# MarwanMousa/MARL-for-IM

Hardware: NVIDIA B200
Metric: agent_steps_per_sec (higher is better)
Workload: dtype i32 state / f64 obs+reward

## Files before the change

### marl_for_im_b200/csrc/imx_api.cu

```cuda
#include <cmath>
#include <cstdarg>
#include <cstdio>
#include <cstdlib>
#include <cstring>
#include <atomic>
#include <new>
#include <vector>

#include <nvtx3/nvToolsExt.h>

#include "imx_reset.cuh"
#include "imx_step_tma.cuh"
#include "imx_rollout.cuh"
#include "imx_step_pipe.cuh"
#include "imx_rollout_et.cuh"
#include "imx_kernels.cuh"
#include "imx_stats.cuh"
#include "imx_jit.cuh"
#include "imx_cc.cuh"
#include "imx_eval.cuh"

using namespace imx;

static thread_local char g_err[512] = "";
// ... 34 lines not shown
        a.message.ascii = name;
        return &a;
    }
};
#define IMX_NVTX(name) NvtxRange nvtx_range__(name)

extern "C" const char* imx_last_error(void) { return g_err; }
extern "C" int imx_abi_version(void) { return IMX_ABI_VERSION; }
extern "C" int imx_config_size(void) { return (int)sizeof(imx_config); }
extern "C" int64_t imx_launch_count(void) { return g_launches.load(); }

typedef void (*reset_fn_t)(const StepArgs, const ResetArgs, int);

struct imx_env {
    imx_config cfg;
    bool div, multi;
    int m, T, P, D, O, L, NB, R, maxc;
    int demand_max[IMX_MAX_NODES];
    int depth[IMX_MAX_NODES], parent[IMX_MAX_NODES], child_slot[IMX_MAX_NODES];
    int retailers[IMX_MAX_NODES], retailer_idx[IMX_MAX_NODES];
    double sell[IMX_MAX_NODES], buy[IMX_MAX_NODES];
    bool need_hd, need_ho, write_hd, has_carry;
    int S;
    int64_t N;
    NodeParams* d_nodes = nullptr;
    int32_t* d_state = nullptr;
    size_t state_bytes = 0;
    void* field_ptr[IMX_F_COUNT] = {};
    int64_t field_cnt[IMX_F_COUNT] = {};
    int32_t* d_err = nullptr;
    int32_t* d_demand_T = nullptr;
    uint8_t* d_mask_T = nullptr;
    double* d_cdf = nullptr;
    uint16_t* d_guide = nullptr;
    int cdf_len = 0;
    double* d_stats_partial = nullptr;
    double* d_dfo_rewards = nullptr;
    double* d_tab = nullptr;
    int TL = 0;
    cudaStream_t hstream = nullptr;
    double *d_act_h = nullptr, *d_obs_h = nullptr, *d_rew_h = nullptr;
    int32_t* d_dem_h = nullptr;
    uint8_t* d_mask_h = nullptr;
    int t = 0;
    int noisy_now = 0;
    uint64_t episode = 0;
    step_fn_t step_fn = nullptr;
    tma_fn_t tma_fn = nullptr;
    tma_fn_t tma_many_fn = nullptr;
    TileLayout tile = {};
    TileLayout tile_jit = {};
    int step_path = 0;
    int host_zero_copy = 1;
    int step_dense = 0;
    int tma_threads = 256;
    int use_pdl = 1;
    int fuse_periods = 1;
    int l2_hints = 0;
    int step_et = 0;
    int rollout_et = 0;
    int jit_threads = 128;
    int pipe_mode = 0;
    int pipe_stages = 0;
    int pipe_ctas = 0;
    int sm_count = 148;
    int jit_policy = 0;
    int jit_state = 0;
    const imxjit::Kernels* jit = nullptr;
    const imxjit::Kernels* jit_noobs = nullptr;
    int jit_noobs_state = 0;
    const imxjit::Kernels* jit_cc = nullptr;
    int jit_cc_state = 0;
    TileLayout tile_cc = {};
    void* d_obs_scratch = nullptr;
    const imxjit::Kernels* jit_ep = nullptr;
    const imxjit::Kernels* jit_ep_noobs = nullptr;
    int jit_ep_state = 0, jit_ep_noobs_state = 0;
    double* d_ep_rewards = nullptr;
    double* d_ep_profit = nullptr;
    double* d_ep_ret = nullptr;
    double* d_ep_stats = nullptr;
    int last_variant = 0;
    reset_fn_t reset_fn = nullptr;
    rollout_fn_t rollout_fn = nullptr;
    int step_grid_cap = 0, rollout_grid_cap = 0;
    size_t step_smem = 0;
    int m_pad = 0;
};

static int obs_type_of(const imx_config& c) { return (c.io_flags & IMX_IO_OBS_BF16) ? OBS_BF16 : c.obs_f32 ? OBS_F32 : OBS_F64; }
static int obs_elem_bytes(const imx_env* e) { return imx::obs_elem_bytes(obs_type_of(e->cfg)); }
static int act_elem_bytes(const imx_env* e) { return (e->cfg.io_flags & IMX_IO_ACTIONS_F32) ? 4 : 8; }
static int64_t bytes_per_env(const imx_env* e) {
    return 8 * (int64_t)e->S + 4 * e->R + (int64_t)e->m * (act_elem_bytes(e) + 8 + e->O * obs_elem_bytes(e));
}

#define IMX_DECL_PICK(MP, DV) void imx_pick_kernels_##MP##_##DV(bool small, bool few, imx::KernelSet* ks);
IMX_DECL_PICK(2, 0) IMX_DECL_PICK(4, 0) IMX_DECL_PICK(8, 0) IMX_DECL_PICK(16, 0) IMX_DECL_PICK(32, 0)
IMX_DECL_PICK(4, 1) IMX_DECL_PICK(8, 1) IMX_DECL_PICK(16, 1) IMX_DECL_PICK(32, 1)
#undef IMX_DECL_PICK

static int m_pad_of(const imx_env* e);
static void pick_kernels(imx_env* e, int m_pad, bool div) {
    const bool small = (e->D <= 4 && e->P <= 1);
    const bool few = e->maxc <= 2;
    KernelSet ks;
    if (div) {
        if (m_pad == 4) imx_pick_kernels_4_1(small, few, &ks);
        else if (m_pad == 8) imx_pick_kernels_8_1(small, few, &ks);
        else if (m_pad == 16) imx_pick_kernels_16_1(small, few, &ks);
        else imx_pick_kernels_32_1(small, few, &ks);
    } else {
        if (m_pad == 2) imx_pick_kernels_2_0(small, few, &ks);
        else if (m_pad == 4) imx_pick_kernels_4_0(small, few, &ks);
        else if (m_pad == 8) imx_pick_kernels_8_0(small, few, &ks);
        else if (m_pad == 16) imx_pick_kernels_16_0(small, few, &ks);
        else imx_pick_kernels_32_0(small, few, &ks);
    }
    e->step_fn = ks.step_fn; e->tma_fn = ks.tma_fn; e->tma_many_fn = ks.tma_many_fn; e->rollout_fn = ks.rollout_fn;
    const int ot = obs_type_of(e->cfg);
    if (ot == OBS_BF16) e->reset_fn = small ? reset_kernel<4, 1, OBS_BF16> : reset_kernel<8, 8, OBS_BF16>;
    else if (ot == OBS_F32) e->reset_fn = small ? reset_kernel<4, 1, OBS_F32> : reset_kernel<8, 8, OBS_F32>;
    else e->reset_fn = small ? reset_kernel<4, 1, OBS_F64> : reset_kernel<8, 8, OBS_F64>;
    e->m_pad = m_pad;
}

static cudaError_t raise_dyn_smem_limit(const void* fn, size_t bytes) {
    cudaFuncAttributes fa;
    cudaError_t rc = cudaFuncGetAttributes(&fa, fn);
    if (rc != cudaSuccess) return rc;
    if ((size_t)fa.maxDynamicSharedSizeBytes >= bytes) return cudaSuccess;
    return cudaFuncSetAttribute(fn, cudaFuncAttributeMaxDynamicSharedMemorySize, (int)bytes);
}

static int m_pad_of(const imx_env* e);

static int choose_tma_threads(const imx_env* e) {
    const char* tt = getenv("IMX_TMA_THREADS");
    const bool small4 = !e->div && m_pad_of(e) == 4 && e->N >= 1024 && bytes_per_env(e) * e->N <= ((int64_t)192 << 20);
    const bool big4 = !e->div && m_pad_of(e) == 4 && e->N >= ((int64_t)1 << 19);
    const int dflt = small4 ? 64 : (big4 || (m_pad_of(e) <= 4 && e->N >= ((int64_t)1 << 20))) ? 256 : 128;
    const int v = tt ? atoi(tt) : dflt;
    return ((v == 64 || v == 128 || v == 256 || v == 512) && v >= 2 * m_pad_of(e)) ? v : 256;
}

static int m_pad_of(const imx_env* e) {
    const int m = e->m;
    if (e->div) return m <= 4 ? 4 : m <= 8 ? 8 : m <= 16 ? 16 : 32;
    return m <= 2 ? 2 : m <= 4 ? 4 : m <= 8 ? 8 : m <= 16 ? 16 : 32;
}

static void compute_tile(const imx_env* e, TileLayout& L, int tile_width, bool with_cc = false, int E_fixed = 0) {
    const int m = e->m;
    const int E = E_fixed > 0 ? E_fixed : (e->tma_threads / 32) * (32 / tile_width);
    int off = 0;
    auto take = [&](int bytes) { const int o = off; off += (bytes + 127) & ~127; return o; };
    L.E = E;
    const int act_region = E * m * (act_elem_bytes(e) == 4 ? 12 : 8);
    L.off_act = take(act_region);
    L.off_inv = take(E * m * 4);
    L.off_bl = take(E * m * 4);
    L.off_ou = take(E * m * 4);
    L.off_pipe = take(E * e->L * 4);
    L.off_hd = take(e->need_hd ? E * m * e->P * 4 : 0);
    L.off_ho = take(e->need_ho ? E * m * e->P * 4 : 0);
    L.off_carry = take(e->has_carry ? E * m * 4 : 0);
// ... 646 lines not shown
            IMX_CREATE_CUDA(cudaMemcpy(reinterpret_cast<float*>(e->d_tab + tab.size()) + tab.size(), tabh.data(), tab.size() * sizeof(uint16_t),
                                       cudaMemcpyHostToDevice));
        }
    }
    {
        const int cols = e->multi ? m : 1;
        const int64_t nslices = (N + stats_envs_per_block(cols) - 1) / stats_envs_per_block(cols);
        const size_t a = (size_t)(2 + 2 * cols) * (size_t)nslices, b = (size_t)(2 * EVAL_FIXED + 2 + 2 * IMX_MAX_NODES) * STATS_BLOCKS;
        IMX_CREATE_CUDA(cudaMalloc(&e->d_stats_partial, (a > b ? a : b) * sizeof(double)));
    }
    IMX_CREATE_CUDA(cudaMemset(e->d_demand_T, 0, dem_bytes));
    {
        launch_reset_kernel(e, nullptr, nullptr);
        cudaError_t le = cudaGetLastError();
        if (le != cudaSuccess) { fail(-3, "reset launch failed: %s", cudaGetErrorString(le)); imx_destroy(e); return -3; }
        g_launches.fetch_add(1);
        IMX_CREATE_CUDA(cudaDeviceSynchronize());
    }
#undef IMX_CREATE_CUDA
    ensure_jit(e);
    *out = e;
    return 0;
}

extern "C" int imx_destroy(imx_env* e) {
    if (!e) return 0;
    cudaSetDevice(e->cfg.device);
    if (e->hstream) { cudaStreamSynchronize(e->hstream); cudaStreamDestroy(e->hstream); }
    cudaFree(e->d_nodes); cudaFree(e->d_state); cudaFree(e->d_err);
    cudaFree(e->d_demand_T); cudaFree(e->d_mask_T); cudaFree(e->d_cdf); cudaFree(e->d_guide); cudaFree(e->d_tab); cudaFree(e->d_stats_partial);
    cudaFree(e->d_dfo_rewards); cudaFree(e->d_obs_scratch);
    cudaFree(e->d_ep_rewards); cudaFree(e->d_ep_profit); cudaFree(e->d_ep_ret); cudaFree(e->d_ep_stats);
    cudaFree(e->d_act_h); cudaFree(e->d_obs_h); cudaFree(e->d_rew_h); cudaFree(e->d_dem_h); cudaFree(e->d_mask_h);
    delete e;
    return 0;
}

extern "C" int imx_obs_len(const imx_env* e) { return e ? e->O : fail(-1, "null env"); }
extern "C" int imx_state_words(const imx_env* e) { return e ? e->S : fail(-1, "null env"); }
extern "C" int imx_num_retailers(const imx_env* e) { return e ? e->R : fail(-1, "null env"); }
extern "C" int imx_pipe_words(const imx_env* e) { return e ? e->L : fail(-1, "null env"); }
extern "C" int imx_ledger_words(const imx_env* e) { return e ? e->NB : fail(-1, "null env"); }
extern "C" int imx_retailers(const imx_env* e, int32_t* out) {
    if (!e || !out) return fail(-1, "null argument");
    for (int k = 0; k < e->R; ++k) out[k] = e->retailers[k];
    return 0;
}
extern "C" int imx_demand_max(const imx_env* e, int32_t* out) {
    if (!e || !out) return fail(-1, "null argument");
    for (int i = 0; i < e->m; ++i) out[i] = e->demand_max[i];
    return 0;
}
extern "C" int imx_node_price(const imx_env* e, double* sell, double* buy) {
    if (!e || !sell || !buy) return fail(-1, "null argument");
    for (int i = 0; i < e->m; ++i) { sell[i] = e->sell[i]; buy[i] = e->buy[i]; }
    return 0;
}
extern "C" int imx_state_field(imx_env* e, int field, void** dev_ptr, int64_t* count) {
    if (!e || !dev_ptr || !count) return fail(-1, "null argument");
    if (field < 0 || field >= IMX_F_COUNT) return fail(-1, "unknown field %d", field);
    *dev_ptr = e->field_ptr[field];
    *count = e->field_cnt[field];
    return 0;
}
extern "C" int imx_period(const imx_env* e) { return e ? e->t : fail(-1, "null env"); }
extern "C" int imx_set_period(imx_env* e, int t) {
    if (!e) return fail(-1, "null env");
    if (t < 0 || t > e->T) return fail(-1, "period %d outside [0, %d]", t, e->T);
    e->t = t;
    return 0;
}

static void launch_reset_kernel(imx_env* e, double* obs_dev, cudaStream_t s, const int32_t* demand_in) {
    StepArgs A;
    fill_args(e, A);
    A.obs = obs_dev;
    ResetArgs Z;
    Z.zero_base = e->d_state;
    Z.zero_words = (int64_t)(e->state_bytes / sizeof(int32_t));
    Z.err = e->d_err;
    Z.demand_in = demand_in;
    Z.demand_T = e->d_demand_T;
    Z.R = e->R; Z.T = e->T;
    const int64_t work = (obs_dev ? e->N * e->m * e->O : 0) > Z.zero_words / 4 ? e->N * e->m * e->O : Z.zero_words / 4;
    int sms = 148;
    cudaDeviceGetAttribute(&sms, cudaDevAttrMultiProcessorCount, e->cfg.device);
    int64_t blocks = (work + 255) / 256;
    if (blocks > (int64_t)sms * 8) blocks = (int64_t)sms * 8;
    if (blocks < 1) blocks = 1;
    const size_t smem = (size_t)e->m * e->O * sizeof(double) + (size_t)e->m * sizeof(int32_t);
    cudaLaunchConfig_t lc;
    memset(&lc, 0, sizeof(lc));
    lc.gridDim = dim3((unsigned)blocks); lc.blockDim = dim3(256); lc.dynamicSmemBytes = smem; lc.stream = s;
    cudaLaunchAttribute at[1];
    at[0].id = cudaLaunchAttributeProgrammaticStreamSerialization;
    at[0].val.programmaticStreamSerializationAllowed = 1;
    lc.attrs = at;
    lc.numAttrs = e->use_pdl ? 1 : 0;
    cudaLaunchKernelEx(&lc, e->reset_fn, A, Z, e->div ? 1 : 0);
}

static DemandGen make_gen(const imx_env* e, uint64_t episode) {
    DemandGen g;
    g.dist = e->cfg.demand_dist; g.low = e->cfg.uniform_low; g.high = e->cfg.uniform_high;
    g.cdf_len = e->cdf_len; g.cdf = e->d_cdf; g.guide = e->d_guide; g.seed = e->cfg.seed; g.episode = episode; g.env_offset = e->cfg.env_offset;
    g.noise_thr = e->div ? e->cfg.noisy_demand_threshold : 0.0;
    return g;
}

extern "C" int imx_reset(imx_env* e, const int32_t* demand_dev, const uint8_t* delay_mask_dev, int noisy,
                         uint64_t episode, void* obs_dev, void* stream) {
    IMX_NVTX("imx_reset");

    if (!e) return fail(-1, "null env");
    cudaStream_t s = (cudaStream_t)stream;
    IMX_CUDA(cudaSetDevice(e->cfg.device));
    if ((noisy || delay_mask_dev) && !e->has_carry) return fail(-1, "noisy delay requested but the env was created with noisy_delay = 0");
    if (!demand_dev && e->cfg.demand_dist == IMX_DIST_REPLAY_ONLY)
        return fail(-1, "reset() without a demand trace needs demand_dist poisson or uniform");
    const int64_t N = e->N;
    const unsigned gb = (unsigned)((N * e->R + 255) / 256);
    if (!demand_dev) {
        demand_generate_kernel<<<gb, 256, 0, s>>>(e->d_demand_T, N, e->R, e->T, make_gen(e, episode));
        IMX_CHECK_LAUNCH("demand_generate_kernel");
    }
    e->noisy_now = (noisy || delay_mask_dev) ? 1 : 0;
    const int64_t cells = N * e->m;
    const unsigned cb = (unsigned)((cells + 255) / 256);
    if (e->noisy_now) {
        if (delay_mask_dev) {
            mask_transpose_kernel<<<cb, 256, 0, s>>>(delay_mask_dev, e->d_mask_T, N, e->m, e->T);
            IMX_CHECK_LAUNCH("mask_transpose_kernel");
        } else {
            mask_generate_kernel<<<cb, 256, 0, s>>>(e->d_mask_T, N, e->m, e->T, e->cfg.seed, e->cfg.env_offset, episode,
                                                    e->cfg.noisy_delay_threshold);
            IMX_CHECK_LAUNCH("mask_generate_kernel");
        }
    }
    e->t = 0;
    e->episode = episode;
    launch_reset_kernel(e, (double*)obs_dev, s, demand_dev);
    IMX_CHECK_LAUNCH("reset_kernel");
    return 0;
}

static bool pipe_pays(const imx_env* e, int n_tiles) {
    (void)n_tiles;
    if (e->step_et) return bytes_per_env(e) * e->N <= ((int64_t)384 << 20);
    if (e->div) return true;
    if (e->l2_hints) return true;
    return bytes_per_env(e) * e->N <= ((int64_t)192 << 20);
}
static int pipe_ctas_for(const imx_env* e, const TileLayout& L) {
    const bool is_cc = (&L == &e->tile_cc);
    int want = 4;
    if (e->pipe_ctas > 0) want = e->pipe_ctas;
    else if (e->step_et && !is_cc) want = 6;
    else if (e->div) want = m_pad_of(e) <= 4 ? 4 : 6;
    else if (e->jit_threads == 64) want = 8;
    const int64_t per_cta = (int64_t)pipe_stages_for(e, L) * L.total + 1024 + 256;
    const int fit = (int)((228 * 1024) / per_cta);
    if (want > fit) want = fit;
    return want < 1 ? 1 : want;
}

struct CcOut { void* dev; int fill; double lo, hi; };
static bool tile_io_whole16(const imx_env* e, const TileLayout& L, bool cc) {
    const int64_t cells = (int64_t)L.E * e->m;
    if ((cells * act_elem_bytes(e)) % 16 != 0 || (cells * e->O * obs_elem_bytes(e)) % 16 != 0) return false;
    return !cc || (cells * ((e->m - 1) * (1 + e->O) + e->O) * obs_elem_bytes(e)) % 16 == 0;
}
constexpr unsigned ET_THREADS_HOST = 128;

// ... 329 lines not shown
        return fail(-1, "rollout without a demand trace needs demand_dist poisson or uniform");
    if ((noisy || delay_mask_dev) && !e->has_carry) return fail(-1, "noisy delay requested but the env was created with noisy_delay = 0");
    cudaStream_t s = (cudaStream_t)stream;
    IMX_CUDA(cudaSetDevice(e->cfg.device));
    if (dfo_dev && !step_reward_dev) {
        if (!e->d_dfo_rewards) {
            if (stream_is_capturing(s)) return fail(-1, "dfo_dev without step_reward_dev under stream capture: call imx_prepare(IMX_PREPARE_DFO) first");
            IMX_CUDA(cudaMalloc(&e->d_dfo_rewards, (size_t)e->T * e->N * sizeof(double)));
        }
        step_reward_dev = e->d_dfo_rewards;
    }
    StepArgs A;
    fill_args(e, A);
    A.t = 0;
    RolloutArgs Rg;
    memset(&Rg, 0, sizeof(Rg));
    Rg.z = z_dev; Rg.z_stride = z_stride; Rg.demand = demand_dev;
    Rg.ret = return_dev; Rg.step_reward = step_reward_dev; Rg.write_state = write_state;
    Rg.mask = delay_mask_dev; Rg.noisy = (noisy || delay_mask_dev) ? 1 : 0; Rg.delay_thr = e->cfg.noisy_delay_threshold;
    Rg.gen = make_gen(e, episode);
    const int epw = 32 / e->m_pad;
    const size_t draw_bytes = (size_t)(ROLLOUT_THREADS / 32) * epw * e->R * ((e->T + 1) & ~1) * sizeof(int32_t);
    const bool coop = (!demand_dev && draw_bytes <= 40 * 1024);
    Rg.coop_demand = coop ? 1 : 0;
    const size_t roll_smem = coop ? draw_bytes : 0;
    const int64_t warp_tiles = (e->N + epw - 1) / epw;
    const int64_t blocks_needed = (warp_tiles + (ROLLOUT_THREADS / 32) - 1) / (ROLLOUT_THREADS / 32);
    const unsigned grid = (unsigned)(blocks_needed < e->rollout_grid_cap ? blocks_needed : e->rollout_grid_cap);
    if (e->jit_state == 1 && e->jit->rollout && e->rollout_et) {
        EtNodeConsts C;
        memset(&C, 0, sizeof(C));
        for (int i = 0; i < e->m; ++i) {
            C.p[i] = e->sell[i]; C.c[i] = e->buy[i]; C.h[i] = e->cfg.stock_cost[i]; C.bc[i] = e->cfg.backlog_cost[i]; C.target[i] = e->cfg.inv_target[i];
        }
        void* params[] = {(void*)&A, (void*)&Rg, (void*)&C};
        const int64_t blocks = (e->N + ET_THREADS_HOST - 1) / ET_THREADS_HOST;
        const int64_t cap = (int64_t)e->sm_count * 16;
        Rg.coop_demand = 0;
        const CUresult cr = imxjit::g_api.LaunchKernel(e->jit->rollout, (unsigned)(blocks < cap ? blocks : cap), 1, 1, ET_THREADS_HOST, 1, 1, 0, (CUstream)s,
                                                       params, nullptr);
        if (cr != CUDA_SUCCESS) return fail(-3, "launch of the env-per-thread rollout kernel failed (CUresult %d)", (int)cr);
        g_launches.fetch_add(1, std::memory_order_relaxed);
        e->last_variant = 2;
    } else if (e->jit_state == 1 && e->jit->rollout) {
        void* params[] = {(void*)&A, (void*)&Rg};
        const int epw_j = 32 / e->m;
        const int64_t wt_j = (e->N + epw_j - 1) / epw_j;
        const int64_t need_j = (wt_j + (ROLLOUT_THREADS / 32) - 1) / (ROLLOUT_THREADS / 32);
        const int64_t cap_j = (int64_t)e->rollout_grid_cap * 4;
        const unsigned g2 = (unsigned)(need_j < cap_j ? need_j : cap_j);
        const size_t draw_j = (size_t)(ROLLOUT_THREADS / 32) * epw_j * e->R * ((e->T + 1) & ~1) * sizeof(int32_t);
        if (coop && draw_j > 40 * 1024) Rg.coop_demand = 0;
        const size_t roll_smem_j = Rg.coop_demand ? draw_j : 0;
        const CUresult cr = imxjit::g_api.LaunchKernel(e->jit->rollout, g2, 1, 1, ROLLOUT_THREADS, 1, 1, (unsigned)roll_smem_j, (CUstream)s, params, nullptr);
        if (cr != CUDA_SUCCESS) return fail(-3, "launch of the specialised rollout kernel failed (CUresult %d)", (int)cr);
        g_launches.fetch_add(1, std::memory_order_relaxed);
        e->last_variant = 2;
    } else {
        e->rollout_fn<<<grid, ROLLOUT_THREADS, roll_smem, s>>>(A, Rg);
        IMX_CHECK_LAUNCH("rollout_kernel");
        e->last_variant = 0;
    }
    if (dfo_dev) {
        dfo_objective_kernel<<<(unsigned)((e->N + 127) / 128), 128, 0, s>>>(pmf_dev, step_reward_dev, dfo_dev, e->N, e->R, e->T);
        IMX_CHECK_LAUNCH("dfo_objective_kernel");
    }
    if (write_state) { e->t = e->T; e->episode = episode; e->noisy_now = Rg.noisy; }
    return 0;
}

template <typename... KArgs, typename... Args>
static cudaError_t launch_dependent(void (*kern)(KArgs...), dim3 grid, dim3 block, cudaStream_t s, bool pdl, Args... args) {
    cudaLaunchConfig_t lc;
    memset(&lc, 0, sizeof(lc));
    lc.gridDim = grid; lc.blockDim = block; lc.dynamicSmemBytes = 0; lc.stream = s;
    cudaLaunchAttribute at[1];
    at[0].id = cudaLaunchAttributeProgrammaticStreamSerialization;
    at[0].val.programmaticStreamSerializationAllowed = 1;
    lc.attrs = at;
    lc.numAttrs = pdl ? 1 : 0;
    return cudaLaunchKernelEx(&lc, kern, KArgs(args)...);
}

static int launch_return_stats(imx_env* e, const double* src, int periods, bool fused, double* ret_out, double* stats_dev, int accumulate,
                               cudaStream_t s) {
    const int cols = e->multi ? e->m : 1;
    const int per_agent = e->multi ? 1 : 0;
    const int nstat = per_agent ? 2 + 2 * cols : 2;
    const int epb = stats_envs_per_block(cols);
    const int nslices = (int)((e->N + epb - 1) / epb);
    const bool pdl = e->use_pdl != 0;
    if (fused && periods == 1 && !ret_out) fused = false;
    if (fused)
        IMX_CUDA(launch_dependent(stats_slice_kernel<true>, dim3((unsigned)nslices), dim3(STATS_THREADS), s, pdl, src, ret_out, e->d_stats_partial,
                                  e->N, cols, per_agent, periods, epb, nslices));
    else
        IMX_CUDA(launch_dependent(stats_slice_kernel<false>, dim3((unsigned)nslices), dim3(STATS_THREADS), s, pdl, src, (double*)nullptr,
                                  e->d_stats_partial, e->N, cols, per_agent, 1, epb, nslices));
    g_launches.fetch_add(1, std::memory_order_relaxed);
    IMX_CUDA(launch_dependent(stats_final_kernel, dim3((unsigned)nstat), dim3(STATS_THREADS), s, pdl, (const double*)e->d_stats_partial, stats_dev,
                              e->N, nslices, accumulate));
    g_launches.fetch_add(1, std::memory_order_relaxed);
    return 0;
}

extern "C" int imx_return_stats(imx_env* e, const double* return_dev, double* stats_dev, void* stream) {
    if (!e || !return_dev || !stats_dev) return fail(-1, "null argument");
    IMX_CUDA(cudaSetDevice(e->cfg.device));
    return launch_return_stats(e, return_dev, 1, false, nullptr, stats_dev, 0, (cudaStream_t)stream);
}

extern "C" int imx_episode_stats(imx_env* e, const double* step_reward_dev, int periods, double* return_dev, double* stats_dev,
                                 int accumulate, void* stream) {
    IMX_NVTX("imx_episode_stats");

    if (!e || !step_reward_dev || !stats_dev) return fail(-1, "null argument");
    if (periods < 1) return fail(-1, "periods must be >= 1");
    IMX_CUDA(cudaSetDevice(e->cfg.device));
    return launch_return_stats(e, step_reward_dev, periods, true, return_dev, stats_dev, accumulate, (cudaStream_t)stream);
}

extern "C" int imx_eval_len(const imx_env* e) { return e ? EVAL_FIXED + e->m : -1; }

extern "C" int imx_eval_accumulate(imx_env* e, const void* obs_dev, const double* reward_dev, const double* profit_dev,
                                   double* acc_dev, int reset, void* stream) {
    if (!e || !obs_dev || !reward_dev || !acc_dev) return fail(-1, "null argument");
    IMX_CUDA(cudaSetDevice(e->cfg.device));
    EvalArgs E;
    memset(&E, 0, sizeof(E));
    E.obs = obs_dev; E.reward = reward_dev; E.profit = profit_dev; E.acc = acc_dev; E.nodes = e->d_nodes;
    E.N = e->N; E.m = e->m; E.O = e->O; E.multi = e->multi ? 1 : 0; E.obs_type = obs_type_of(e->cfg);
    E.rescaled = (e->cfg.kind == IMX_KIND_MAIM_DIV || e->cfg.standardise_state) ? 1 : 0;
    E.reset = reset ? 1 : 0;
    E.a = e->cfg.a; E.bma = e->cfg.b - e->cfg.a;
    eval_accumulate_kernel<<<(unsigned)((e->N + 255) / 256), 256, 0, (cudaStream_t)stream>>>(E);
    IMX_CHECK_LAUNCH("eval_accumulate_kernel");
    return 0;
}

extern "C" int imx_eval_stats(imx_env* e, const double* acc_dev, double* stats_dev, int accumulate, void* stream) {
    if (!e || !acc_dev || !stats_dev) return fail(-1, "null argument");
    IMX_CUDA(cudaSetDevice(e->cfg.device));
    const int W = EVAL_FIXED + e->m;
    column_stats_partial_kernel<<<dim3(STATS_BLOCKS, 2 * W), STATS_THREADS, 0, (cudaStream_t)stream>>>(acc_dev, e->d_stats_partial, e->N, W);
    IMX_CHECK_LAUNCH("column_stats_partial_kernel");
    stats_final_kernel<<<2 * W, STATS_THREADS, 0, (cudaStream_t)stream>>>(e->d_stats_partial, stats_dev, e->N, STATS_BLOCKS, accumulate);
    IMX_CHECK_LAUNCH("stats_final_kernel");
    return 0;
}

static int ensure_host_path(imx_env* e) {
    if (e->hstream) return 0;
    const size_t cells = (size_t)e->N * e->m;
    cudaError_t rc = cudaSuccess;
    auto take = [&](void** p, size_t bytes) { if (rc == cudaSuccess && !*p) rc = cudaMalloc(p, bytes); };
    take((void**)&e->d_act_h, cells * sizeof(double));
    take((void**)&e->d_obs_h, cells * e->O * obs_elem_bytes(e));
    take((void**)&e->d_rew_h, cells * sizeof(double));
    take((void**)&e->d_dem_h, (size_t)e->N * e->R * e->T * sizeof(int32_t));
    if (e->has_carry) take((void**)&e->d_mask_h, (size_t)e->N * e->T * e->m);
    cudaStream_t hs = nullptr;
    if (rc == cudaSuccess) rc = cudaStreamCreateWithFlags(&hs, cudaStreamNonBlocking);
    if (rc != cudaSuccess) {
        cudaFree(e->d_act_h); cudaFree(e->d_obs_h); cudaFree(e->d_rew_h); cudaFree(e->d_dem_h); cudaFree(e->d_mask_h);
        e->d_act_h = e->d_obs_h = e->d_rew_h = nullptr; e->d_dem_h = nullptr; e->d_mask_h = nullptr;
        return fail(-2, "host-path staging allocation failed: %s", cudaGetErrorString(rc));
    }
    e->hstream = hs;
    return 0;
}

extern "C" int imx_reset_host(imx_env* e, const int32_t* demand_host, const uint8_t* delay_mask_host, int noisy,
                              uint64_t episode, void* obs_host) {
    IMX_NVTX("imx_reset_host");

    if (!e) return fail(-1, "null env");
    IMX_CUDA(cudaSetDevice(e->cfg.device));
    int rc = ensure_host_path(e);
    if (rc) return rc;
    cudaStream_t s = e->hstream;
    if (demand_host)
// ... 140 lines not shown
```

### marl_for_im_b200/csrc/imx_reset.cuh

```cuda
#pragma once

#include "imx_step.cuh"

namespace imx {

struct ResetArgs {
    int32_t* zero_base;
    int64_t zero_words;
    int32_t* err;
    const int32_t* demand_in;
    int32_t* demand_T;
    int32_t R, T;
};
constexpr int RESET_T_CHUNK = 8;

template <int DMAX, int PMAX, int OT>
__global__ void __launch_bounds__(256) reset_kernel(const __grid_constant__ StepArgs A_, const __grid_constant__ ResetArgs Z, int div) {
    extern __shared__ __align__(16) double s_tmpl[];
    StepArgs A = A_;
    A.obs_type = OT;
    const int m = A.m, O = A.O;
    const int es = obs_elem_bytes(OT);
    int32_t* s_init = reinterpret_cast<int32_t*>(s_tmpl + m * O);
    asm volatile("griddepcontrol.wait;" ::: "memory");
    asm volatile("griddepcontrol.launch_dependents;" ::: "memory");
    if ((int)threadIdx.x < m) {
        const int i = threadIdx.x;
        const NodeParams np = load_node(A.nodes + i);
        s_init[i] = np.init_inv;
        if (A.obs) {
            int pipe[DMAX], hd[PMAX], ho[PMAX];
#pragma unroll
            for (int k = 0; k < DMAX; ++k) pipe[k] = 0;
#pragma unroll
            for (int j = 0; j < PMAX; ++j) { hd[j] = 0; ho[j] = 0; }
            write_obs_row<DMAX, PMAX, true>(reinterpret_cast<unsigned char*>(s_tmpl) + (size_t)i * O * es, A, np, i, A.tab ? A.tab + (size_t)i * 4 * A.TL : nullptr, np.init_inv, 0, 0, pipe, hd,
                                      ho, div != 0);
        }
    }
    const int64_t stride = (int64_t)gridDim.x * blockDim.x;
    const int64_t gtid = (int64_t)blockIdx.x * blockDim.x + threadIdx.x;
    int4* z4 = reinterpret_cast<int4*>(Z.zero_base);
    const int64_t n4 = Z.zero_words / 4;
    for (int64_t k = gtid; k < n4; k += stride) z4[k] = make_int4(0, 0, 0, 0);
    for (int64_t k = n4 * 4 + gtid; k < Z.zero_words; k += stride) Z.zero_base[k] = 0;
    for (int64_t k = gtid; k < A.N; k += stride) Z.err[k] = 0;
    if (Z.demand_in) {
        const int R = Z.R, T = Z.T;
        const int chunks = (T + RESET_T_CHUNK - 1) / RESET_T_CHUNK;
        const int64_t rows = A.N * R;
        const int64_t items = rows * chunks;
        for (int64_t k = gtid; k < items; k += stride) {
            const int ch = (int)(k / rows);
            const int64_t idx = k - (int64_t)ch * rows;
            const int r = (int)(idx / A.N);
            const int64_t n = idx - (int64_t)r * A.N;
            const int32_t* src = Z.demand_in + (n * R + r) * T;
            const int t0 = ch * RESET_T_CHUNK;
            int v[RESET_T_CHUNK];
#pragma unroll
            for (int u = 0; u < RESET_T_CHUNK; ++u) v[u] = (t0 + u < T) ? src[t0 + u] : 0;
#pragma unroll
            for (int u = 0; u < RESET_T_CHUNK; ++u)
                if (t0 + u < T) Z.demand_T[((int64_t)(t0 + u) * R + r) * A.N + n] = v[u];
        }
    }
    __syncthreads();
    if (A.obs) {
        const int64_t bytes = A.N * m * O * es;
        const int tmpl_bytes = m * O * es;
        if ((tmpl_bytes & 15) == 0 && (reinterpret_cast<uintptr_t>(A.obs) & 15) == 0) {
            const int len = tmpl_bytes / 16;
            const int64_t total = bytes / 16;
            const int4* src = reinterpret_cast<const int4*>(s_tmpl);
            int4* dst = reinterpret_cast<int4*>(A.obs);
            const int step = (int)(stride % len);
            int rem = (int)(gtid % len);
            for (int64_t k = gtid; k < total; k += stride) {
                dst[k] = src[rem];
                rem += step;
                if (rem >= len) rem -= len;
            }
        } else {
            const int len = m * O;
            const int64_t total = A.N * len;
            const int step = (int)(stride % len);
            int rem = (int)(gtid % len);
            for (int64_t k = gtid; k < total; k += stride) {
                if (OT == OBS_BF16) reinterpret_cast<uint16_t*>(A.obs)[k] = reinterpret_cast<const uint16_t*>(s_tmpl)[rem];
                else if (OT == OBS_F32) reinterpret_cast<float*>(A.obs)[k] = reinterpret_cast<const float*>(s_tmpl)[rem];
                else A.obs[k] = s_tmpl[rem];
                rem += step;
                if (rem >= len) rem -= len;
            }
        }
    }
    const int64_t cells = A.N * m;
    for (int64_t k = gtid; k < (cells + 3) / 4; k += stride) {
        int rem = (int)((k * 4) % m);
#pragma unroll
        for (int q = 0; q < 4; ++q) {
            const int64_t c = k * 4 + q;
            if (c < cells) A.inv[c] = s_init[rem];
            if (++rem == m) rem = 0;
        }
    }
}

__global__ void __launch_bounds__(256) demand_generate_kernel(int32_t* __restrict__ out, int64_t N, int R, int T, DemandGen g) {
    const int64_t idx = (int64_t)blockIdx.x * blockDim.x + threadIdx.x;
    if (idx >= N * R) return;
    const int r = (int)(idx / N);
    const int64_t n = idx % N;
    for (int t = 0; t < T; t += 2) {
        int d0, d1;
        draw_demand_pair(g, n, r, t, d0, d1);
        out[((int64_t)t * R + r) * N + n] = d0;
        if (t + 1 < T) out[((int64_t)(t + 1) * R + r) * N + n] = d1;
    }
}

__global__ void __launch_bounds__(256) mask_transpose_kernel(const uint8_t* __restrict__ in, uint8_t* __restrict__ out,
                                                             int64_t N, int m, int T) {
    const int64_t cell = (int64_t)blockIdx.x * blockDim.x + threadIdx.x;
    if (cell >= N * m) return;
    const int64_t n = cell / m;
    const int i = (int)(cell % m);
    for (int t = 0; t < T; ++t) out[((int64_t)t * N + n) * m + i] = in[(n * T + t) * m + i];
}

__global__ void __launch_bounds__(256) mask_generate_kernel(uint8_t* __restrict__ out, int64_t N, int m, int T, uint64_t seed,
                                                            int64_t env_offset, uint64_t episode, double thr) {
    const int64_t cell = (int64_t)blockIdx.x * blockDim.x + threadIdx.x;
    if (cell >= N * m) return;
    const int64_t n = cell / m;
    const int i = (int)(cell % m);
    for (int t = 0; t < T; ++t) out[((int64_t)t * N + n) * m + i] = draw_delay(seed, env_offset + n, i, t, episode, thr) ? 1 : 0;
}

}
```

### marl_for_im_b200/csrc/imx_stats.cuh

```cuda
#pragma once

#include "imx_device.cuh"

namespace imx {

struct DfoTerm {
    const double* __restrict__ pmf_row;
    const double* __restrict__ rew;
    int64_t stride;
    int T;
    __device__ __forceinline__ double operator()(int j) const { return __dmul_rn(pmf_row[j], rew[(int64_t)(j % T) * stride]); }
};

__device__ __forceinline__ double np_pairwise_block(const DfoTerm& f, int lo, int n) {
    if (n < 8) {
        double res = 0.0;
        for (int i = 0; i < n; ++i) res = __dadd_rn(res, f(lo + i));
        return res;
    }
    double r[8];
#pragma unroll
    for (int j = 0; j < 8; ++j) r[j] = f(lo + j);
    int i = 8;
    for (; i < n - (n % 8); i += 8) {
#pragma unroll
        for (int j = 0; j < 8; ++j) r[j] = __dadd_rn(r[j], f(lo + i + j));
    }
    double res = __dadd_rn(__dadd_rn(__dadd_rn(r[0], r[1]), __dadd_rn(r[2], r[3])),
                           __dadd_rn(__dadd_rn(r[4], r[5]), __dadd_rn(r[6], r[7])));
    for (; i < n; ++i) res = __dadd_rn(res, f(lo + i));
    return res;
}

__device__ inline double np_pairwise(const DfoTerm& f, int total) {
    struct Frame { int lo, n, stage; double left; };
    Frame st[24];
    int sp = 0;
    double ret = 0.0;
    st[sp].lo = 0; st[sp].n = total; st[sp].stage = 0; st[sp].left = 0.0; ++sp;
    while (sp > 0) {
        const int lo = st[sp - 1].lo, n = st[sp - 1].n, stage = st[sp - 1].stage;
        int n2 = n / 2;
        n2 -= n2 % 8;
        if (stage == 0) {
            if (n <= 128) { ret = np_pairwise_block(f, lo, n); --sp; }
            else { st[sp - 1].stage = 1; st[sp].lo = lo; st[sp].n = n2; st[sp].stage = 0; st[sp].left = 0.0; ++sp; }
        } else if (stage == 1) {
            st[sp - 1].left = ret; st[sp - 1].stage = 2;
            st[sp].lo = lo + n2; st[sp].n = n - n2; st[sp].stage = 0; st[sp].left = 0.0; ++sp;
        } else {
            ret = __dadd_rn(st[sp - 1].left, ret);
            --sp;
        }
    }
    return ret;
}

__global__ void __launch_bounds__(128) dfo_objective_kernel(const double* __restrict__ pmf, const double* __restrict__ step_reward,
                                                            double* __restrict__ dfo, int64_t N, int R, int T) {
    const int64_t n = (int64_t)blockIdx.x * blockDim.x + threadIdx.x;
    if (n >= N) return;
    DfoTerm f;
    f.pmf_row = pmf + n * (int64_t)R * T;
    f.rew = step_reward + n;
    f.stride = N;
    f.T = T;
    const double s = np_pairwise(f, R * T);
    dfo[n] = __dmul_rn(-1.0 / (double)T, s);
}

constexpr int STATS_THREADS = 256;
constexpr int STATS_BLOCKS = 128;

constexpr int STATS_SLICE_CELLS = 1024;
static inline int stats_envs_per_block(int cols) {
    int e = (STATS_SLICE_CELLS / cols) & ~31;
    if (e > STATS_THREADS) e = STATS_THREADS;
    return e < 32 ? 32 : e;
}

__device__ __forceinline__ double warp_sum_fixed(double v) {
#pragma unroll
    for (int off = 16; off > 0; off >>= 1) v = __dadd_rn(v, __shfl_down_sync(0xffffffffu, v, off));
    return v;
}

template <bool FUSED>
__global__ void __launch_bounds__(STATS_THREADS) stats_slice_kernel(const double* __restrict__ src, double* __restrict__ ret_out,
                                                                    double* __restrict__ partial, int64_t N, int cols, int per_agent, int T,
                                                                    int epb, int nslices) {
    __shared__ double s_ret[STATS_SLICE_CELLS + STATS_THREADS];
    constexpr int MAXK = STATS_SLICE_CELLS / STATS_THREADS;
    const int tid = threadIdx.x, lane = tid & 31, warp = tid >> 5;
    const int stride = cols | 1;
    const int64_t env0 = (int64_t)blockIdx.x * epb;
    const int64_t cells = N * cols;
    const int64_t cell0 = env0 * cols;
    const int my_cells = epb * cols;
    asm volatile("griddepcontrol.wait;" ::: "memory");
    asm volatile("griddepcontrol.launch_dependents;" ::: "memory");
    double acc[MAXK];
#pragma unroll
    for (int k = 0; k < MAXK; ++k) {
        const int j = tid + k * STATS_THREADS;
        const int64_t c = cell0 + j;
        acc[k] = 0.0;
        if (j < my_cells && c < cells) {
            if (FUSED) {
                int t = 0;
                for (; t + 10 <= T; t += 10) {
                    double r[10];
#pragma unroll
                    for (int u = 0; u < 10; ++u) r[u] = src[(int64_t)(t + u) * cells + c];
#pragma unroll
                    for (int u = 0; u < 10; ++u) acc[k] = __dadd_rn(acc[k], r[u]);
                }
                for (; t < T; ++t) acc[k] = __dadd_rn(acc[k], src[(int64_t)t * cells + c]);
                if (ret_out) ret_out[c] = acc[k];
            } else {
                acc[k] = src[c];
            }
        }
    }
#pragma unroll
    for (int k = 0; k < MAXK; ++k) {
        const int j = tid + k * STATS_THREADS;
        if (j < my_cells) s_ret[(j / cols) * stride + (j % cols)] = acc[k];
    }
    __syncthreads();
    const int live = (int)(N - env0 < epb ? N - env0 : epb);
    for (int task = warp; task <= cols; task += STATS_THREADS / 32) {
        if (task < cols && !per_agent) continue;
        double sum = 0.0, sq = 0.0;
        for (int e = lane; e < live; e += 32) {
            double v;
            if (task < cols) {
                v = s_ret[e * stride + task];
            } else {
                v = 0.0;
                for (int c = 0; c < cols; ++c) v = __dadd_rn(v, s_ret[e * stride + c]);
            }
            sum = __dadd_rn(sum, v);
            sq = __dadd_rn(sq, __dmul_rn(v, v));
        }
        sum = warp_sum_fixed(sum);
        sq = warp_sum_fixed(sq);
        if (lane == 0) {
            const int q = task < cols ? 2 + 2 * task : 0;
            partial[(int64_t)q * nslices + blockIdx.x] = sum;
            partial[(int64_t)(q + 1) * nslices + blockIdx.x] = sq;
        }
    }
}

__global__ void __launch_bounds__(STATS_THREADS) stats_final_kernel(const double* __restrict__ partial, double* __restrict__ stats, int64_t N,
                                                                   int nslices, int accumulate) {
    __shared__ double red[STATS_THREADS];
    const int q = blockIdx.x;
    asm volatile("griddepcontrol.wait;" ::: "memory");
    double acc = 0.0;
    for (int b = threadIdx.x; b < nslices; b += STATS_THREADS) acc += partial[(int64_t)q * nslices + b];
    red[threadIdx.x] = acc;
    __syncthreads();
    for (int s = STATS_THREADS / 2; s >= 32; s >>= 1) {
        if ((int)threadIdx.x < s) red[threadIdx.x] += red[threadIdx.x + s];
        __syncthreads();
    }
    if (threadIdx.x < 32) {
        const double v = warp_sum_fixed(red[threadIdx.x]);
        if (threadIdx.x == 0) {
            stats[1 + q] = accumulate ? stats[1 + q] + v : v;
            if (q == 0) stats[0] = accumulate ? stats[0] + (double)N : (double)N;
        }
    }
}

}
```

Measured before the change: 39.18 billion.

## Use bulk async smem-to-global copies for reset obs fill and retune stats slice

The reset kernel now builds a replicated observation template run in shared memory and streams it to global memory with cp.async.bulk stores, optionally using an L2 evict-first hint, in place of per-thread int4 stores. The reset grid is sized from an occupancy query instead of a fixed 8 CTAs per SM. The fused stats slice kernel is templated on thread count and load-unroll depth, interleaving loads across all cells per thread for more memory-level parallelism, with the shape selectable by environment variable and defaulting to 512x6. This adds template instantiations and relies on the asynchronous bulk copies being fully drained before the kernel exits.

```diff
diff --git a/marl_for_im_b200/csrc/imx_api.cu b/marl_for_im_b200/csrc/imx_api.cu
--- a/marl_for_im_b200/csrc/imx_api.cu
+++ b/marl_for_im_b200/csrc/imx_api.cu
@@ -140,6 +140,7 @@
     double* d_ep_stats = nullptr;
     int last_variant = 0;
     reset_fn_t reset_fn = nullptr;
+    int reset_ctas = 0;
     rollout_fn_t rollout_fn = nullptr;
     int step_grid_cap = 0, rollout_grid_cap = 0;
     size_t step_smem = 0;
@@ -952,13 +953,20 @@
     Z.demand_in = demand_in;
     Z.demand_T = e->d_demand_T;
     Z.R = e->R; Z.T = e->T;
+    const int tmpl_bytes = e->m * e->O * obs_elem_bytes(e);
+    Z.tmpl_rep = reset_tmpl_rep(tmpl_bytes);
+    Z.obs_evict_first = e->l2_hints ? 1 : 0;
     const int64_t work = (obs_dev ? e->N * e->m * e->O : 0) > Z.zero_words / 4 ? e->N * e->m * e->O : Z.zero_words / 4;
-    int sms = 148;
-    cudaDeviceGetAttribute(&sms, cudaDevAttrMultiProcessorCount, e->cfg.device);
+    const size_t smem = reset_smem_bytes(e->m, e->O, tmpl_bytes);
+    if (!e->reset_ctas) {
+        int sms = 148, occ = RESET_MIN_CTAS;
+        cudaDeviceGetAttribute(&sms, cudaDevAttrMultiProcessorCount, e->cfg.device);
+        cudaOccupancyMaxActiveBlocksPerMultiprocessor(&occ, (const void*)e->reset_fn, 256, smem);
+        e->reset_ctas = sms * (occ > 0 ? occ : 1);
+    }
     int64_t blocks = (work + 255) / 256;
-    if (blocks > (int64_t)sms * 8) blocks = (int64_t)sms * 8;
+    if (blocks > (int64_t)e->reset_ctas) blocks = e->reset_ctas;
     if (blocks < 1) blocks = 1;
-    const size_t smem = (size_t)e->m * e->O * sizeof(double) + (size_t)e->m * sizeof(int32_t);
     cudaLaunchConfig_t lc;
     memset(&lc, 0, sizeof(lc));
     lc.gridDim = dim3((unsigned)blocks); lc.blockDim = dim3(256); lc.dynamicSmemBytes = smem; lc.stream = s;
@@ -1454,6 +1462,27 @@
     return cudaLaunchKernelEx(&lc, kern, KArgs(args)...);
 }
 
+using StatsSliceFn = void (*)(const double*, double*, double*, int64_t, int, int, int, int, int);
+struct StatsShape { int threads, lif; StatsSliceFn fn; };
+static const StatsShape STATS_SHAPES[] = {
+    {512, 6, stats_slice_kernel<true, 512, 6>},
+    {256, 4, stats_slice_kernel<true, 256, 4>},   {256, 8, stats_slice_kernel<true, 256, 8>},
+    {512, 4, stats_slice_kernel<true, 512, 4>},   {512, 8, stats_slice_kernel<true, 512, 8>},
+    {1024, 4, stats_slice_kernel<true, 1024, 4>}, {1024, 8, stats_slice_kernel<true, 1024, 8>},
+    {1024, 10, stats_slice_kernel<true, 1024, 10>},
+};
+static const StatsShape& stats_shape() {
+    static const StatsShape* pick = [] {
+        const char* v = getenv("IMX_STATS_SHAPE");
+        int th = 0, lif = 0;
+        if (v && sscanf(v, "%dx%d", &th, &lif) == 2)
+            for (const StatsShape& sh : STATS_SHAPES)
+                if (sh.threads == th && sh.lif == lif) return &sh;
+        return &STATS_SHAPES[0];
+    }();
+    return *pick;
+}
+
 static int launch_return_stats(imx_env* e, const double* src, int periods, bool fused, double* ret_out, double* stats_dev, int accumulate,
                                cudaStream_t s) {
     const int cols = e->multi ? e->m : 1;
@@ -1463,12 +1492,14 @@
     const int nslices = (int)((e->N + epb - 1) / epb);
     const bool pdl = e->use_pdl != 0;
     if (fused && periods == 1 && !ret_out) fused = false;
-    if (fused)
-        IMX_CUDA(launch_dependent(stats_slice_kernel<true>, dim3((unsigned)nslices), dim3(STATS_THREADS), s, pdl, src, ret_out, e->d_stats_partial,
+    if (fused) {
+        const StatsShape& sh = stats_shape();
+        IMX_CUDA(launch_dependent(sh.fn, dim3((unsigned)nslices), dim3((unsigned)sh.threads), s, pdl, src, ret_out, e->d_stats_partial,
                                   e->N, cols, per_agent, periods, epb, nslices));
-    else
-        IMX_CUDA(launch_dependent(stats_slice_kernel<false>, dim3((unsigned)nslices), dim3(STATS_THREADS), s, pdl, src, (double*)nullptr,
-                                  e->d_stats_partial, e->N, cols, per_agent, 1, epb, nslices));
+    } else {
+        IMX_CUDA(launch_dependent(stats_slice_kernel<false, STATS_THREADS, 1>, dim3((unsigned)nslices), dim3(STATS_THREADS), s, pdl, src,
+                                  (double*)nullptr, e->d_stats_partial, e->N, cols, per_agent, 1, epb, nslices));
+    }
     g_launches.fetch_add(1, std::memory_order_relaxed);
     IMX_CUDA(launch_dependent(stats_final_kernel, dim3((unsigned)nstat), dim3(STATS_THREADS), s, pdl, (const double*)e->d_stats_partial, stats_dev,
                               e->N, nslices, accumulate));
diff --git a/marl_for_im_b200/csrc/imx_reset.cuh b/marl_for_im_b200/csrc/imx_reset.cuh
--- a/marl_for_im_b200/csrc/imx_reset.cuh
+++ b/marl_for_im_b200/csrc/imx_reset.cuh
@@ -11,31 +11,82 @@
     const int32_t* demand_in;
     int32_t* demand_T;
     int32_t R, T;
+    int32_t tmpl_rep;
+    int32_t obs_evict_first;
 };
 constexpr int RESET_T_CHUNK = 8;
+constexpr int RESET_MIN_CTAS = 5;
+constexpr int RESET_RUN_BYTES = 4096;
+
+static inline int reset_tmpl_rep(int tmpl_bytes) {
+    if (tmpl_bytes <= 0 || (tmpl_bytes & 15) != 0) return 1;
+    return RESET_RUN_BYTES / tmpl_bytes > 1 ? RESET_RUN_BYTES / tmpl_bytes : 1;
+}
+static inline size_t reset_smem_bytes(int m, int O, int tmpl_bytes) {
+    const size_t run = (size_t)reset_tmpl_rep(tmpl_bytes) * tmpl_bytes, build = (size_t)m * O * sizeof(double);
+    return (((size_t)m * sizeof(int32_t) + 15) & ~(size_t)15) + (run > build ? run : build);
+}
+
+__device__ __forceinline__ uint64_t reset_policy_evict_first() {
+    uint64_t p;
+    asm volatile("createpolicy.fractional.L2::evict_first.b64 %0, 1.0;" : "=l"(p));
+    return p;
+}
+__device__ __forceinline__ void reset_bulk_store(void* gdst, uint32_t s, uint32_t bytes, bool evict_first, uint64_t policy) {
+    if (evict_first)
+        asm volatile("cp.async.bulk.global.shared::cta.bulk_group.L2::cache_hint [%0], [%1], %2, %3;" ::"l"(gdst), "r"(s), "r"(bytes),
+                     "l"(policy)
+                     : "memory");
+    else
+        asm volatile("cp.async.bulk.global.shared::cta.bulk_group [%0], [%1], %2;" ::"l"(gdst), "r"(s), "r"(bytes) : "memory");
+}
 
 template <int DMAX, int PMAX, int OT>
-__global__ void __launch_bounds__(256) reset_kernel(const __grid_constant__ StepArgs A_, const __grid_constant__ ResetArgs Z, int div) {
-    extern __shared__ __align__(16) double s_tmpl[];
+__global__ void __launch_bounds__(256, RESET_MIN_CTAS) reset_kernel(const __grid_constant__ StepArgs A_, const __grid_constant__ ResetArgs Z, int div) {
+    extern __shared__ __align__(16) int32_t s_init[];
     StepArgs A = A_;
     A.obs_type = OT;
     const int m = A.m, O = A.O;
     const int es = obs_elem_bytes(OT);
-    int32_t* s_init = reinterpret_cast<int32_t*>(s_tmpl + m * O);
+    unsigned char* s_tmpl = reinterpret_cast<unsigned char*>(s_init) + ((m * 4 + 15) & ~15);
+    const int tmpl_bytes = m * O * es;
+    const bool bulk = A.obs && (tmpl_bytes & 15) == 0 && (reinterpret_cast<uintptr_t>(A.obs) & 15) == 0;
     asm volatile("griddepcontrol.wait;" ::: "memory");
     asm volatile("griddepcontrol.launch_dependents;" ::: "memory");
-    if ((int)threadIdx.x < m) {
+    if (threadIdx.x < 32) {
         const int i = threadIdx.x;
-        const NodeParams np = load_node(A.nodes + i);
-        s_init[i] = np.init_inv;
-        if (A.obs) {
-            int pipe[DMAX], hd[PMAX], ho[PMAX];
+        if (i < m) {
+            const NodeParams np = load_node(A.nodes + i);
+            s_init[i] = np.init_inv;
+            if (A.obs) {
+                int pipe[DMAX], hd[PMAX], ho[PMAX];
 #pragma unroll
-            for (int k = 0; k < DMAX; ++k) pipe[k] = 0;
+                for (int k = 0; k < DMAX; ++k) pipe[k] = 0;
 #pragma unroll
-            for (int j = 0; j < PMAX; ++j) { hd[j] = 0; ho[j] = 0; }
-            write_obs_row<DMAX, PMAX, true>(reinterpret_cast<unsigned char*>(s_tmpl) + (size_t)i * O * es, A, np, i, A.tab ? A.tab + (size_t)i * 4 * A.TL : nullptr, np.init_inv, 0, 0, pipe, hd,
-                                      ho, div != 0);
+                for (int j = 0; j < PMAX; ++j) { hd[j] = 0; ho[j] = 0; }
+                write_obs_row<DMAX, PMAX, true>(s_tmpl + (size_t)i * O * es, A, np, i, A.tab ? A.tab + (size_t)i * 4 * A.TL : nullptr, np.init_inv, 0, 0,
+                                                pipe, hd, ho, div != 0);
+            }
+        }
+        if (bulk) {
+            __syncwarp();
+            const int len = tmpl_bytes / 16, rep = Z.tmpl_rep;
+            int4* run = reinterpret_cast<int4*>(s_tmpl);
+            for (int q = len + i; q < rep * len; q += 32) run[q] = run[q % len];
+            fence_proxy_async_smem();
+            __syncwarp();
+            if (i == 0) {
+                const int64_t e0 = A.N * blockIdx.x / gridDim.x, e1 = A.N * (blockIdx.x + 1) / gridDim.x;
+                const int64_t total = (e1 - e0) * tmpl_bytes;
+                const int64_t chunk = (int64_t)rep * tmpl_bytes;
+                unsigned char* dst = reinterpret_cast<unsigned char*>(A.obs) + e0 * tmpl_bytes;
+                const uint32_t src = (uint32_t)__cvta_generic_to_shared(s_tmpl);
+                const bool ef = Z.obs_evict_first != 0;
+                const uint64_t policy = ef ? reset_policy_evict_first() : 0;
+                for (int64_t off = 0; off < total; off += chunk)
+                    reset_bulk_store(dst + off, src, (uint32_t)(total - off < chunk ? total - off : chunk), ef, policy);
+                asm volatile("cp.async.bulk.commit_group;" ::: "memory");
+            }
         }
     }
     const int64_t stride = (int64_t)gridDim.x * blockDim.x;
@@ -66,33 +117,17 @@
         }
     }
     __syncthreads();
-    if (A.obs) {
-        const int64_t bytes = A.N * m * O * es;
-        const int tmpl_bytes = m * O * es;
-        if ((tmpl_bytes & 15) == 0 && (reinterpret_cast<uintptr_t>(A.obs) & 15) == 0) {
-            const int len = tmpl_bytes / 16;
-            const int64_t total = bytes / 16;
-            const int4* src = reinterpret_cast<const int4*>(s_tmpl);
-            int4* dst = reinterpret_cast<int4*>(A.obs);
-            const int step = (int)(stride % len);
-            int rem = (int)(gtid % len);
-            for (int64_t k = gtid; k < total; k += stride) {
-                dst[k] = src[rem];
-                rem += step;
-                if (rem >= len) rem -= len;
-            }
-        } else {
-            const int len = m * O;
-            const int64_t total = A.N * len;
-            const int step = (int)(stride % len);
-            int rem = (int)(gtid % len);
-            for (int64_t k = gtid; k < total; k += stride) {
-                if (OT == OBS_BF16) reinterpret_cast<uint16_t*>(A.obs)[k] = reinterpret_cast<const uint16_t*>(s_tmpl)[rem];
-                else if (OT == OBS_F32) reinterpret_cast<float*>(A.obs)[k] = reinterpret_cast<const float*>(s_tmpl)[rem];
-                else A.obs[k] = s_tmpl[rem];
-                rem += step;
-                if (rem >= len) rem -= len;
-            }
+    if (A.obs && !bulk) {
+        const int len = m * O;
+        const int64_t total = A.N * len;
+        const int step = (int)(stride % len);
+        int rem = (int)(gtid % len);
+        for (int64_t k = gtid; k < total; k += stride) {
+            if (OT == OBS_BF16) reinterpret_cast<uint16_t*>(A.obs)[k] = reinterpret_cast<const uint16_t*>(s_tmpl)[rem];
+            else if (OT == OBS_F32) reinterpret_cast<float*>(A.obs)[k] = reinterpret_cast<const float*>(s_tmpl)[rem];
+            else A.obs[k] = reinterpret_cast<const double*>(s_tmpl)[rem];
+            rem += step;
+            if (rem >= len) rem -= len;
         }
     }
     const int64_t cells = A.N * m;
@@ -105,6 +140,7 @@
             if (++rem == m) rem = 0;
         }
     }
+    if (bulk && threadIdx.x == 0) bulk_wait_read_all();
 }
 
 __global__ void __launch_bounds__(256) demand_generate_kernel(int32_t* __restrict__ out, int64_t N, int R, int T, DemandGen g) {
diff --git a/marl_for_im_b200/csrc/imx_stats.cuh b/marl_for_im_b200/csrc/imx_stats.cuh
--- a/marl_for_im_b200/csrc/imx_stats.cuh
+++ b/marl_for_im_b200/csrc/imx_stats.cuh
@@ -85,12 +85,12 @@
     return v;
 }
 
-template <bool FUSED>
-__global__ void __launch_bounds__(STATS_THREADS) stats_slice_kernel(const double* __restrict__ src, double* __restrict__ ret_out,
-                                                                    double* __restrict__ partial, int64_t N, int cols, int per_agent, int T,
-                                                                    int epb, int nslices) {
+template <bool FUSED, int THREADS, int LIF>
+__global__ void __launch_bounds__(THREADS, FUSED ? 2 : 8) stats_slice_kernel(const double* __restrict__ src, double* __restrict__ ret_out,
+                                                                 double* __restrict__ partial, int64_t N, int cols, int per_agent, int T,
+                                                                 int epb, int nslices) {
     __shared__ double s_ret[STATS_SLICE_CELLS + STATS_THREADS];
-    constexpr int MAXK = STATS_SLICE_CELLS / STATS_THREADS;
+    constexpr int MAXK = STATS_SLICE_CELLS / THREADS;
     const int tid = threadIdx.x, lane = tid & 31, warp = tid >> 5;
     const int stride = cols | 1;
     const int64_t env0 = (int64_t)blockIdx.x * epb;
@@ -101,35 +101,45 @@
     asm volatile("griddepcontrol.launch_dependents;" ::: "memory");
     double acc[MAXK];
 #pragma unroll
-    for (int k = 0; k < MAXK; ++k) {
-        const int j = tid + k * STATS_THREADS;
-        const int64_t c = cell0 + j;
-        acc[k] = 0.0;
-        if (j < my_cells && c < cells) {
-            if (FUSED) {
-                int t = 0;
-                for (; t + 10 <= T; t += 10) {
-                    double r[10];
+    for (int k = 0; k < MAXK; ++k) acc[k] = 0.0;
+    if (FUSED) {
+        bool live_cell[MAXK];
 #pragma unroll
-                    for (int u = 0; u < 10; ++u) r[u] = src[(int64_t)(t + u) * cells + c];
+        for (int k = 0; k < MAXK; ++k) live_cell[k] = tid + k * THREADS < my_cells && cell0 + tid + k * THREADS < cells;
+        for (int t = 0; t < T; t += LIF) {
+            double r[MAXK][LIF];
 #pragma unroll
-                    for (int u = 0; u < 10; ++u) acc[k] = __dadd_rn(acc[k], r[u]);
-                }
-                for (; t < T; ++t) acc[k] = __dadd_rn(acc[k], src[(int64_t)t * cells + c]);
-                if (ret_out) ret_out[c] = acc[k];
-            } else {
-                acc[k] = src[c];
-            }
+            for (int k = 0; k < MAXK; ++k)
+#pragma unroll
+                for (int u = 0; u < LIF; ++u)
+                    r[k][u] = (live_cell[k] && t + u < T) ? src[(int64_t)(t + u) * cells + cell0 + tid + k * THREADS] : 0.0;
+#pragma unroll
+            for (int k = 0; k < MAXK; ++k)
+#pragma unroll
+                for (int u = 0; u < LIF; ++u)
+                    if (t + u < T) acc[k] = __dadd_rn(acc[k], r[k][u]);
+        }
+        if (ret_out) {
+#pragma unroll
+            for (int k = 0; k < MAXK; ++k)
+                if (live_cell[k]) ret_out[cell0 + tid + k * THREADS] = acc[k];
+        }
+    } else {
+#pragma unroll
+        for (int k = 0; k < MAXK; ++k) {
+            const int j = tid + k * THREADS;
+            const int64_t c = cell0 + j;
+            if (j < my_cells && c < cells) acc[k] = src[c];
         }
     }
 #pragma unroll
     for (int k = 0; k < MAXK; ++k) {
-        const int j = tid + k * STATS_THREADS;
+        const int j = tid + k * THREADS;
         if (j < my_cells) s_ret[(j / cols) * stride + (j % cols)] = acc[k];
     }
     __syncthreads();
     const int live = (int)(N - env0 < epb ? N - env0 : epb);
-    for (int task = warp; task <= cols; task += STATS_THREADS / 32) {
+    for (int task = warp; task <= cols; task += THREADS / 32) {
         if (task < cols && !per_agent) continue;
         double sum = 0.0, sq = 0.0;
         for (int e = lane; e < live; e += 32) {
```

Measured after the change: 39.81 billion, median of 6. 1.6% higher.
